# zendesk/min-tfs-client

Hardware: AMD Instinct MI355X
Metric: predict_req_per_s (higher is better)
Workload: dtype fp32; 1 GPU; model=identity-echo[resnet50], global_batch=32, parallelism=dp1, pipeline=4, encoding=turbo, grpc_impl=native, copy_mode=1, streaming=auto, transport=unix, servers_per_rank=1, gpu=True

## Files before the change

min_tfs_client_amd/ops/csrc/grpc_transport.cpp:

```cpp
#include <pybind11/eval.h>
#include <pybind11/functional.h>
#include <pybind11/pybind11.h>
#include <pybind11/stl.h>
#include <torch/extension.h>

#include <c10/hip/HIPCachingAllocator.h>
#include <c10/hip/HIPGuard.h>
#include <c10/hip/HIPStream.h>

#include <algorithm>
#include <atomic>
#include <chrono>
#include <condition_variable>
#include <cstring>
#include <deque>
#include <map>
#include <memory>
#include <mutex>
#include <set>
#include <string>
#include <thread>
#include <unordered_map>
#include <vector>

#include "h2core.h"
#include "hpack.h"
#include "staging.h"
#include "wire.h"

namespace py = pybind11;

namespace {

using h2::Buf;
using h2::Conn;
using h2::ConnError;
using h2::FrameHeader;

struct WireRegion {
  size_t offset;
  size_t nbytes;
  uintptr_t ptr;
  bool device;
};

void write_message_with_regions(Conn& conn, uint32_t stream,
                                const uint8_t* buf, size_t len,
                                const std::vector<WireRegion>& regions,
                                bool end_stream) {
  h2::DataMessageWriter w(conn, stream, len, end_stream);
  size_t pos = 0;
  for (const auto& r : regions) {
    if (r.offset < pos || r.nbytes > len || r.offset > len - r.nbytes)
      throw ConnError("bad streaming region");
    if (r.offset > pos) w.write(buf + pos, r.offset - pos);
    if (!r.device) {
      w.write(reinterpret_cast<const uint8_t*>(r.ptr), r.nbytes);
    } else {
      mi355x_staging::Lease lease;
      lease.ctx->d2h(reinterpret_cast<const void*>(r.ptr), r.nbytes,
                     [&w](const void* chunk, size_t n) {
                       w.write(static_cast<const uint8_t*>(chunk), n);
                     });
    }
    pos = r.offset + r.nbytes;
  }
  if (pos < len) w.write(buf + pos, len - pos);
  w.finish();
}

bool extract_streaming_reply(py::handle result,
                             std::unique_ptr<py::buffer_info>* info,
                             const uint8_t** buf, size_t* len,
                             std::vector<WireRegion>* regions) {
  if (!py::hasattr(result, "_wire_regions")) return false;
  py::object buffer = result.attr("buffer");
  *info = std::make_unique<py::buffer_info>(py::buffer(buffer).request());
  *buf = static_cast<const uint8_t*>((*info)->ptr);
  *len = size_t((*info)->size) * size_t((*info)->itemsize);
  for (auto item : result.attr("_wire_regions")) {
    auto t = py::reinterpret_borrow<py::tuple>(item);
    regions->push_back(WireRegion{
        t[0].cast<size_t>(), t[1].cast<size_t>(),
        uintptr_t(t[2].cast<uint64_t>()), t[3].cast<bool>()});
  }
  return true;
}

struct RpcCallError : std::runtime_error {
  int code;
  RpcCallError(int code_, const std::string& msg)
      : std::runtime_error(msg), code(code_) {}
// ... 121 lines not shown
class ProspectStreams {
 public:
  static ProspectStreams& instance() {
    static ProspectStreams* p = new ProspectStreams();
    return *p;
  }

  static constexpr int kPerDevice = 4;

  hipStream_t get(int device) {
    std::lock_guard<std::mutex> lk(mu_);
    auto it = per_dev_.find(device);
    if (it == per_dev_.end()) {
      std::vector<hipStream_t> v;
      if (hipSetDevice(device) == hipSuccess) {
        for (int i = 0; i < kPerDevice; ++i) {
          hipStream_t s = nullptr;
          if (hipStreamCreateWithFlags(&s, hipStreamNonBlocking) !=
              hipSuccess)
            break;
          v.push_back(s);
        }
      }
      it = per_dev_.emplace(device, std::move(v)).first;
    }
    if (it->second.empty()) return nullptr;
    return it->second[rr_++ % it->second.size()];
  }

 private:
  std::mutex mu_;
  std::unordered_map<int, std::vector<hipStream_t>> per_dev_;
  size_t rr_ = 0;
};

struct DeviceParse {
  bool enabled = false;
  bool failed = false;
  bool done = false;
  int device = 0;
  hipStream_t stream = nullptr;
  int spec_field = 2;
  int map_field = 1;
  std::string spec_name, spec_signature, spec_label;
  int64_t spec_version = -1;
  std::vector<std::string> out_filter;
  std::function<bool(const std::string&)> skip_model;
  size_t pos = 0;
  int state = 0;
  size_t entry_end = 0, tp_end = 0;
  std::string cur_name;
  int cur_dtype = 0;
  std::vector<int64_t> cur_shape;
  bool cur_has_tensor = false;
  at::Tensor cur_tensor;
  bool in_content = false;
  size_t content_off = 0, content_len = 0, content_copied = 0;
  bool copies_issued = false;
  std::vector<std::pair<std::string, at::Tensor>> outs;

  static constexpr size_t kCopyBatch = 1u << 20;

  void fail() {
    failed = true;
    in_content = false;
  }

  void quiesce() {
    if (copies_issued && stream != nullptr) {
      (void)hipStreamSynchronize(stream);
      copies_issued = false;
    }
  }

  DeviceParse() = default;
  DeviceParse(const DeviceParse&) = delete;
  DeviceParse& operator=(const DeviceParse&) = delete;
  DeviceParse(DeviceParse&& o) noexcept { *this = std::move(o); }
  DeviceParse& operator=(DeviceParse&& o) noexcept {
    if (this != &o) {
      quiesce();
      enabled = o.enabled; failed = o.failed; done = o.done;
      device = o.device; stream = o.stream;
      spec_field = o.spec_field; map_field = o.map_field;
      spec_name = std::move(o.spec_name);
      spec_signature = std::move(o.spec_signature);
      spec_label = std::move(o.spec_label);
      spec_version = o.spec_version;
      out_filter = std::move(o.out_filter);
      skip_model = std::move(o.skip_model);
      pos = o.pos; state = o.state;
      entry_end = o.entry_end; tp_end = o.tp_end;
      cur_name = std::move(o.cur_name);
      cur_dtype = o.cur_dtype;
      cur_shape = std::move(o.cur_shape);
      cur_has_tensor = o.cur_has_tensor;
      cur_tensor = std::move(o.cur_tensor);
      in_content = o.in_content;
      content_off = o.content_off;
      content_len = o.content_len;
      content_copied = o.content_copied;
      copies_issued = o.copies_issued;
      outs = std::move(o.outs);
      o.copies_issued = false;
      o.enabled = false;
      o.stream = nullptr;
    }
    return *this;
  }
  ~DeviceParse() { quiesce(); }
};

struct MsgAssembly {
  uint8_t prefix[5];
  size_t prefix_have = 0;
  Buf msg;
  size_t msg_have = 0;
  bool have_len = false;

  void feed_from_socket(int fd, size_t n) {
    while (n > 0) {
      if (prefix_have < 5) {
        size_t take = 5 - prefix_have < n ? 5 - prefix_have : n;
        h2::read_full(fd, prefix + prefix_have, take);
        prefix_have += take;
        n -= take;
        if (prefix_have == 5) {
          if (prefix[0] != 0)
            throw RpcCallError(GRPC_UNIMPLEMENTED,
                               "compressed gRPC messages not supported");
          uint32_t len = h2::be32(prefix + 1);
          if (len > (1u << 30))
            throw RpcCallError(
                GRPC_RESOURCE_EXHAUSTED,
                "received message larger than max (" +
                    std::to_string(len) + " vs 1073741824)");
          size_t cap = 0;
          auto& pool = PinnedPool::instance();
          uint8_t* pinned = pool.get(len, &cap);
          if (pinned != nullptr)
            msg.adopt(pinned, cap, &PinnedPool::deleter, &pool);
          else
            msg.alloc(len);
          msg.len = len;
          have_len = true;
        }
        continue;
      }
      if (!have_len || msg_have + n > msg.len)
        throw ConnError("DATA overruns gRPC message length");
      h2::read_full(fd, msg.p + msg_have, n);
      msg_have += n;
      n = 0;
    }
  }

  bool complete() const { return have_len && msg_have == msg.len; }
};

inline void device_parse_advance(DeviceParse& dp, MsgAssembly& body) {
  if (!dp.enabled || dp.failed || dp.done) return;
  if (!body.have_len) return;
  if (dp.pos == 0 && dp.outs.empty() && !dp.in_content) {
    if (body.msg.deleter == nullptr || body.msg.len < (1u << 20)) {
      dp.enabled = false;
      return;
    }
  }
  const uint8_t* base = body.msg.p;
  const size_t watermark = body.msg_have;
  const size_t total = body.msg.len;

  auto issue_copies = [&]() -> bool {
    size_t span_end = dp.content_off + dp.content_len;
    size_t have_end = watermark < span_end ? watermark : span_end;
    size_t done_abs = dp.content_off + dp.content_copied;
    if (have_end > done_abs) {
      size_t n = have_end - done_abs;
      bool flush = have_end == span_end || body.complete();
      if (n >= DeviceParse::kCopyBatch || flush) {
        if (hipSetDevice(dp.device) != hipSuccess) { dp.fail(); return false; }
        char* dst = static_cast<char*>(dp.cur_tensor.data_ptr())
                    + dp.content_copied;
        if (hipMemcpyAsync(dst, base + done_abs, n, hipMemcpyHostToDevice,
                           dp.stream) != hipSuccess) {
          dp.fail();
          return false;
        }
        dp.copies_issued = true;
        dp.content_copied += n;
      }
    }
    return dp.content_copied == dp.content_len;
  };

  try {
    while (true) {
      if (dp.in_content) {
// ... 62 lines not shown
            tfswire::Cursor v = c.read_len_delim();
            dp.out_filter.emplace_back(
                reinterpret_cast<const char*>(v.p), size_t(v.end - v.p));
            dp.pos = size_t(c.p - base);
          } else {
            dp.fail();
            return;
          }
        } else if (dp.state == 1) {
          int wt = 0;
          int f = c.read_tag(&wt);
          if (f != 1 || wt != tfswire::WT_LEN) { dp.fail(); return; }
          tfswire::Cursor key = c.read_len_delim();
          dp.cur_name.assign(reinterpret_cast<const char*>(key.p),
                             size_t(key.end - key.p));
          f = c.read_tag(&wt);
          if (f != 2 || wt != tfswire::WT_LEN) { dp.fail(); return; }
          uint64_t len = c.read_varint();
          size_t body_off = size_t(c.p - base);
          if (body_off + len > dp.entry_end) { dp.fail(); return; }
          dp.tp_end = body_off + len;
          dp.pos = body_off;
          dp.state = 2;
          dp.cur_dtype = 0;
          dp.cur_shape.clear();
          dp.cur_has_tensor = false;
          dp.cur_tensor = at::Tensor();
        } else {
          if (dp.pos == dp.tp_end) {
            if (!dp.cur_has_tensor) {
              int64_t numel = 1;
              for (int64_t d : dp.cur_shape) numel *= d;
              at::ScalarType st;
              if (numel == 0 && tf_dtype_to_scalar(dp.cur_dtype, &st)) {
                c10::hip::HIPStreamGuard g(c10::hip::getStreamFromExternal(
                    dp.stream, static_cast<c10::DeviceIndex>(dp.device)));
                dp.cur_tensor = at::empty(
                    dp.cur_shape, at::TensorOptions().dtype(st).device(
                                      at::kCUDA, dp.device));
                dp.cur_has_tensor = true;
              } else {
                dp.fail();
                return;
              }
            }
            dp.outs.emplace_back(dp.cur_name, dp.cur_tensor);
            dp.cur_tensor = at::Tensor();
            if (dp.pos != dp.entry_end) { dp.fail(); return; }
            dp.state = 0;
            continue;
          }
          int wt = 0;
          int f = c.read_tag(&wt);
          if (f == 1 && wt == tfswire::WT_VARINT) {
            dp.cur_dtype = int(c.read_varint());
          } else if (f == 2 && wt == tfswire::WT_LEN) {
            tfswire::Cursor sh = c.read_len_delim();
            dp.cur_shape.clear();
            while (!sh.done()) {
              int swt = 0;
              int sf = sh.read_tag(&swt);
              if (sf == 2 && swt == tfswire::WT_LEN) {
                tfswire::Cursor dim = sh.read_len_delim();
                int64_t size = 0;
                while (!dim.done()) {
                  int dwt = 0;
                  int df = dim.read_tag(&dwt);
                  if (df == 1 && dwt == tfswire::WT_VARINT)
                    size = int64_t(dim.read_varint());
                  else
                    dim.skip(dwt);
                }
                dp.cur_shape.push_back(size);
              } else if (sf == 3) {
                dp.fail();
                return;
              } else {
                sh.skip(swt);
              }
            }
          } else if (f == 3 && wt == tfswire::WT_VARINT) {
            (void)c.read_varint();
          } else if (f == 4 && wt == tfswire::WT_LEN) {
            uint64_t len = c.read_varint();
            size_t off = size_t(c.p - base);
            if (off + len > dp.tp_end) { dp.fail(); return; }
            at::ScalarType st;
            if (!tf_dtype_to_scalar(dp.cur_dtype, &st)) { dp.fail(); return; }
            int64_t numel = 1;
            for (int64_t d : dp.cur_shape) numel *= d;
            size_t esize = at::elementSize(st);
            if (uint64_t(numel) * esize != len) { dp.fail(); return; }
            {
              c10::hip::HIPStreamGuard g(c10::hip::getStreamFromExternal(
                  dp.stream, static_cast<c10::DeviceIndex>(dp.device)));
              dp.cur_tensor = at::empty(
                  dp.cur_shape,
                  at::TensorOptions().dtype(st).device(at::kCUDA,
                                                       dp.device));
            }
            dp.content_off = off;
            dp.content_len = size_t(len);
            dp.content_copied = 0;
            dp.in_content = true;
            dp.pos = off;
            continue;
          } else {
            dp.fail();
            return;
          }
          dp.pos = size_t(c.p - base);
        }
      } catch (const std::exception&) {
        (void)step_start;
        if (body.complete()) dp.fail();
        return;
      }
    }
  } catch (...) {
    dp.fail();
  }
}

struct HeaderBlock {
  std::string block;
  bool end_stream = false;
// ... 841 lines not shown
      std::string block = make_request_headers(path, timeout_s);
      try {
        conn_->send_headers(id, block, false);
      } catch (const std::exception& e) {
        pending_.erase(id);
        conn_->close_send_stream(id);
        throw RpcCallError(GRPC_UNAVAILABLE, e.what());
      }
    }
    return id;
  }

  uint32_t start_call(const std::string& path, const uint8_t* data,
                      size_t len, double timeout_s) {
    uint32_t id = begin_stream(path, timeout_s);
    try {
      conn_->send_data_message(id, data, len, true);
    } catch (const std::exception& e) {
      std::lock_guard<std::mutex> lk(mu_);
      pending_.erase(id);
      conn_->close_send_stream(id);
      throw RpcCallError(GRPC_UNAVAILABLE, e.what());
    }
    return id;
  }

  hipStream_t device_stream(int dev) {
    return ProspectStreams::instance().get(dev);
  }

  uint32_t start_call_streaming(const std::string& path, const uint8_t* buf,
                                size_t len,
                                const std::vector<WireRegion>& regions,
                                double timeout_s, int parse_device = -1) {
    uint32_t id = begin_stream(path, timeout_s);
    if (parse_device >= 0) {
      hipStream_t ds = device_stream(parse_device);
      if (ds != nullptr) {
        auto p = find_pending(id);
        if (p) {
          std::lock_guard<std::mutex> lk(p->m);
          p->dparse.enabled = true;
          p->dparse.device = parse_device;
          p->dparse.stream = ds;
        }
      }
    }
    try {
      write_message_with_regions(*conn_, id, buf, len, regions, true);
    } catch (const std::exception& e) {
      std::lock_guard<std::mutex> lk(mu_);
      pending_.erase(id);
      conn_->close_send_stream(id);
      throw RpcCallError(GRPC_UNAVAILABLE, e.what());
    }
    return id;
  }

  struct ParsedResult {
    Buf resp;
    bool parsed_ok = false;
    std::vector<std::pair<std::string, at::Tensor>> outs;
  };

  ParsedResult wait_parsed(uint32_t id, double timeout_s) {
    std::shared_ptr<Pending> p;
    {
      std::lock_guard<std::mutex> lk(mu_);
      auto it = pending_.find(id);
      if (it == pending_.end())
        throw RpcCallError(GRPC_INTERNAL, "unknown call handle");
      p = it->second;
    }
    auto quiesce = [&] {
      std::lock_guard<std::mutex> lk(p->m);
      if (p->dparse.enabled && p->dparse.stream != nullptr)
        (void)hipStreamSynchronize(p->dparse.stream);
    };
    std::unique_lock<std::mutex> lk(p->m);
    bool ok = true;
    if (timeout_s > 0) {
      ok = p->cv.wait_for(lk, std::chrono::duration<double>(timeout_s),
                          [&] { return p->done; });
    } else {
      p->cv.wait(lk, [&] { return p->done; });
    }
    if (!ok) {
      lk.unlock();
      quiesce();
      {
        std::lock_guard<std::mutex> glk(mu_);
        pending_.erase(id);
      }
      try {
        conn_->send_rst_stream(id, 8 );
      } catch (...) {
      }
      conn_->close_send_stream(id);
      cv_.notify_all();
      throw RpcCallError(GRPC_DEADLINE_EXCEEDED, "Deadline Exceeded");
    }
    ParsedResult r;
    r.resp = std::move(p->body.msg);
    int status = p->grpc_status;
    std::string msg = p->message;
    bool parsed = p->dparse.enabled && !p->dparse.failed && p->dparse.done;
    if (parsed) r.outs = std::move(p->dparse.outs);
    bool need_sync = p->dparse.enabled && p->dparse.stream != nullptr;
    hipStream_t ds = p->dparse.stream;
    lk.unlock();
    if (need_sync && hipStreamSynchronize(ds) != hipSuccess) parsed = false;
    if (parsed) record_consumer_stream(r.outs, r.outs.empty() ? 0 :
        r.outs.front().second.get_device());
    {
      std::lock_guard<std::mutex> glk(mu_);
      pending_.erase(id);
    }
    conn_->close_send_stream(id);
    cv_.notify_all();
    if (status != GRPC_OK)
      throw RpcCallError(status < 0 ? GRPC_INTERNAL : status, msg);
    r.parsed_ok = parsed;
    return r;
  }

  Buf wait(uint32_t id, double timeout_s) {
    std::shared_ptr<Pending> p;
    {
      std::lock_guard<std::mutex> lk(mu_);
      auto it = pending_.find(id);
      if (it == pending_.end())
        throw RpcCallError(GRPC_INTERNAL, "unknown call handle");
      p = it->second;
    }
    std::unique_lock<std::mutex> lk(p->m);
    bool ok = true;
    if (timeout_s > 0) {
      ok = p->cv.wait_for(lk, std::chrono::duration<double>(timeout_s),
                          [&] { return p->done; });
    } else {
      p->cv.wait(lk, [&] { return p->done; });
    }
    if (!ok) {
      lk.unlock();
      {
        std::lock_guard<std::mutex> glk(mu_);
        pending_.erase(id);
      }
      try {
        conn_->send_rst_stream(id, 8 );
      } catch (...) {
      }
      conn_->close_send_stream(id);
      cv_.notify_all();
      throw RpcCallError(GRPC_DEADLINE_EXCEEDED, "Deadline Exceeded");
    }
// ... 194 lines not shown
          }
          case h2::F_WINDOW_UPDATE: {
            uint8_t buf4[4];
            if (fh.length != 4) throw ConnError("bad WINDOW_UPDATE");
            h2::read_full(conn_->fd, buf4, 4);
            conn_->apply_window_update(fh.stream,
                                       h2::be32(buf4) & 0x7fffffff);
            break;
          }
          case h2::F_RST_STREAM: {
            uint8_t buf4[4];
            if (fh.length != 4) throw ConnError("bad RST_STREAM");
            h2::read_full(conn_->fd, buf4, 4);
            auto p = find_pending(fh.stream);
            if (p)
              complete(p, GRPC_UNAVAILABLE,
                       "stream reset by server (http2 code " +
                           std::to_string(h2::be32(buf4)) + ")");
            break;
          }
          case h2::F_GOAWAY:
          default:
            h2::discard(conn_->fd, fh.length);
            break;
        }
      }
    } catch (const std::exception& e) {
      conn_->mark_broken(e.what());
      fail_all_pending(GRPC_UNAVAILABLE,
                       std::string("connection lost: ") + e.what());
    }
  }
};

}


PYBIND11_MODULE(_transport, m) {
  m.doc() = "Native gRPC (HTTP/2) transport for the MI355X serving stack";

  py::class_<OwnedBuf>(m, "OwnedBuf", py::buffer_protocol())
      .def_buffer([](OwnedBuf& b) -> py::buffer_info {
        return py::buffer_info(b.buf.p, 1,
                               py::format_descriptor<uint8_t>::format(),
                               1, {py::ssize_t(b.buf.len)}, {py::ssize_t(1)},
                               true );
      })
      .def("__len__", [](const OwnedBuf& b) { return b.buf.len; })
      .def("tobytes", [](const OwnedBuf& b) {
        return py::bytes(reinterpret_cast<const char*>(b.buf.p), b.buf.len);
      });

  static py::object rpc_error_cls = [&m]() {
    py::dict ns;
    py::exec(R"(
class NativeRpcError(Exception):
    """gRPC call failure from the native transport (code_int, details)."""
    def __init__(self, code, details):
        super().__init__(code, details)
        self.code_int = code
        self.details = details
)",
             ns, ns);
    py::object cls = ns["NativeRpcError"];
    m.attr("NativeRpcError") = cls;
    return cls;
// ... 149 lines not shown
                  t[0].cast<size_t>(), t[1].cast<size_t>(),
                  uintptr_t(t[2].cast<uint64_t>()), t[3].cast<bool>()});
            }
            py::gil_scoped_release release;
            return ch.start_call_streaming(path, ptr, len, regions,
                                           timeout, parse_device);
          },
          py::arg("path"), py::arg("data"), py::arg("regions"),
          py::arg("timeout") = 0.0, py::arg("parse_device") = -1,
          "Streaming-region variant of start(); the send completes before "
          "this returns (region memory may be released), the response is "
          "collected with wait().")
      .def(
          "start",
          [](GrpcChannel& ch, const std::string& path, py::buffer data,
             double timeout) {
            py::buffer_info info = data.request();
            const uint8_t* ptr = static_cast<const uint8_t*>(info.ptr);
            size_t len = size_t(info.size) * size_t(info.itemsize);
            py::gil_scoped_release release;
            return ch.start_call(path, ptr, len, timeout);
          },
          py::arg("path"), py::arg("data"), py::arg("timeout") = 0.0)
      .def(
          "wait",
          [](GrpcChannel& ch, uint32_t id, double timeout) {
            py::gil_scoped_release release;
            Buf resp = ch.wait(id, timeout);
            return OwnedBuf(std::move(resp));
          },
          py::arg("id"), py::arg("timeout") = 0.0)
      .def("close", &GrpcChannel::close,
           py::call_guard<py::gil_scoped_release>());
}
```

min_tfs_client_amd/ops/csrc/staging.h:

```cpp
#pragma once

#include <hip/hip_runtime_api.h>

#include <chrono>
#include <condition_variable>
#include <cstdint>
#include <cstdio>
#include <cstdlib>
#include <cstring>
#include <mutex>
#include <stdexcept>
#include <string>
#include <utility>
#include <vector>

namespace mi355x_staging {

#define MI355X_STAGING_CHECK(expr)                                       \
  do {                                                                   \
    hipError_t _e = (expr);                                              \
    if (_e != hipSuccess)                                                \
      throw std::runtime_error(std::string("HIP error in staging: ") +   \
                               hipGetErrorString(_e) + " at " #expr);    \
  } while (0)

inline size_t chunk_size() {
  static const size_t v = [] {
    const char* e = std::getenv("MI355X_STAGING_CHUNK");
    long long n = e ? std::atoll(e) : 0;
    if (n < (1 << 20) || n > (32 << 20)) n = 4 << 20;
    return size_t(n);
  }();
  return v;
}
constexpr int kMaxCtx = 8;

struct Ctx {
  hipStream_t stream = nullptr;
  void* buf[2] = {nullptr, nullptr};
  hipEvent_t evt[2] = {};
  hipEvent_t producer_evt = {};

  void init() {
    MI355X_STAGING_CHECK(
        hipStreamCreateWithFlags(&stream, hipStreamNonBlocking));
    for (int i = 0; i < 2; ++i) {
      MI355X_STAGING_CHECK(hipHostMalloc(&buf[i], chunk_size()));
      MI355X_STAGING_CHECK(
          hipEventCreateWithFlags(&evt[i], hipEventDisableTiming));
    }
    MI355X_STAGING_CHECK(
        hipEventCreateWithFlags(&producer_evt, hipEventDisableTiming));
  }

  void wait_producer(hipStream_t producer) {
    MI355X_STAGING_CHECK(hipEventRecord(producer_evt, producer));
    MI355X_STAGING_CHECK(hipStreamWaitEvent(stream, producer_evt, 0));
  }

  template <typename Consume>
  void d2h(const void* src_dev, size_t nbytes, Consume&& consume) {
    const size_t kChunk = chunk_size();
    size_t nchunks = (nbytes + kChunk - 1) / kChunk;
    const char* trace_path = std::getenv("MI355X_STAGING_TRACE");
    std::vector<double> wait_ms, consume_ms;
    size_t issued = 0;
    for (size_t c = 0; c < (nchunks < 2 ? nchunks : 2); ++c) {
      size_t off = c * kChunk;
      size_t len = nbytes - off < kChunk ? nbytes - off : kChunk;
      MI355X_STAGING_CHECK(hipMemcpyAsync(
          buf[c & 1], static_cast<const char*>(src_dev) + off, len,
          hipMemcpyDeviceToHost, stream));
      MI355X_STAGING_CHECK(hipEventRecord(evt[c & 1], stream));
      ++issued;
    }
    for (size_t c = 0; c < nchunks; ++c) {
      size_t off = c * kChunk;
      size_t len = nbytes - off < kChunk ? nbytes - off : kChunk;
      std::chrono::steady_clock::time_point t0, t1, t2;
      if (trace_path) t0 = std::chrono::steady_clock::now();
      MI355X_STAGING_CHECK(hipEventSynchronize(evt[c & 1]));
      if (trace_path) t1 = std::chrono::steady_clock::now();
      consume(static_cast<const void*>(buf[c & 1]), len);
      if (trace_path) {
        t2 = std::chrono::steady_clock::now();
        wait_ms.push_back(
            std::chrono::duration<double, std::milli>(t1 - t0).count());
        consume_ms.push_back(
            std::chrono::duration<double, std::milli>(t2 - t1).count());
      }
// ... 99 lines not shown
```

min_tfs_client_amd/turbo.py:

```python
from __future__ import annotations

import os
from typing import Dict, Optional, Union

import grpc

try:
    import torch
except ImportError:
    torch = None

from .ops import require_native
from .utils.allocator import tune_malloc
from .utils.metrics import MetricsRegistry
from .utils.tracing import trace_span

_PREDICT_PATH = "/tensorflow.serving.PredictionService/Predict"

_CHANNEL_OPTS = [
    ("grpc.max_send_message_length", 1 << 30),
    ("grpc.max_receive_message_length", 1 << 30),
    ("grpc.http2.max_frame_size", 16 * 1024 * 1024 - 1),
]


def _identity(x: bytes) -> bytes:
    return x


_INT_TO_STATUS = {code.value[0]: code for code in grpc.StatusCode}


class NativeRpcError(grpc.RpcError):

# ... 156 lines not shown
        targets = [target] if isinstance(target, str) else list(target)
        n = max(len(targets), max(1, num_channels))
        self._channels = []
        self._stubs = []
        if backend == "native":
            if credentials is not None:
                raise ValueError("backend='native' is cleartext (h2c); use "
                                 "backend='grpcio' for TLS")
            from . import _transport
            for i in range(n):
                ch = _transport.GrpcChannel(targets[i % len(targets)])
                self._channels.append(ch)
                self._stubs.append(_NativeStub(ch, _PREDICT_PATH))
        elif backend == "grpcio":
            opts = _CHANNEL_OPTS + (options or [])
            for i in range(n):
                copts = opts + [("grpc.use_local_subchannel_pool", 1),
                                ("grpc.channel_id", i)]
                tgt = targets[i % len(targets)]
                if credentials:
                    ch = grpc.secure_channel(tgt, credentials,
                                             options=copts)
                else:
                    ch = grpc.insecure_channel(tgt, options=copts)
                self._channels.append(ch)
                self._stubs.append(ch.unary_unary(
                    _PREDICT_PATH, request_serializer=_identity,
                    response_deserializer=_identity))
        else:
            raise ValueError(f"unknown backend {backend!r}")
        self._channel = self._channels[0]
        self._predict = self._stubs[0]
        self._rr = 0
        self.metrics = MetricsRegistry()
        self.__send_pool = None

    @property
    def _send_pool(self):
        if self.__send_pool is None:
            from concurrent.futures import ThreadPoolExecutor
            self.__send_pool = ThreadPoolExecutor(
                max_workers=16, thread_name_prefix="turbo-send")
        return self.__send_pool

    def _next_stub(self):
        stub = self._stubs[self._rr % len(self._stubs)]
        self._rr += 1
        return stub

    def close(self):
        if self.__send_pool is not None:
            self.__send_pool.shutdown(wait=False)
            self.__send_pool = None
        for ch in self._channels:
            ch.close()

    def __enter__(self):
        return self

    def __exit__(self, *exc):
        self.close()

    def serialize_request(self, model_name: str,
                          inputs: Dict[str, "torch.Tensor"],
                          model_version: Optional[int] = None,
                          signature_name: str = "",
# ... 138 lines not shown
                                signature_name, output_device, copy_mode,
                                streaming=streaming)
        keys = list(inputs.keys())
        if any(inputs[k].dim() == 0 for k in keys):
            return self.predict(model_name, inputs, timeout, model_version,
                                signature_name, output_device, copy_mode,
                                streaming=streaming)
        batch = inputs[keys[0]].shape[0]
        if any(inputs[k].shape[0] != batch for k in keys) \
                or batch < shards:
            return self.predict(model_name, inputs, timeout, model_version,
                                signature_name, output_device, copy_mode,
                                streaming=streaming)
        base, rem = divmod(batch, shards)
        sizes = [base + (1 if i < rem else 0) for i in range(shards)]
        use_streaming = (self.backend == "native" if streaming is None
                         else streaming)
        if use_streaming and self.backend != "native":
            raise ValueError("streaming=True requires backend='native'")

        shard_views = []
        off = 0
        for n in sizes:
            shard_views.append({k: inputs[k].narrow(0, off, n)
                                for k in keys})
            off += n

        dev = str(output_device) if output_device is not None else "cpu"
        parse_dev = -1
        if (use_streaming and dev.startswith("cuda") and torch is not None
                and os.environ.get("MI355X_RX_PARSE", "1") != "0"):
            parse_dev = torch.device(dev).index or 0

        def send_shard(i):
            shard = shard_views[i]
            stub = self._stubs[i % len(self._stubs)]
            if use_streaming:
                blob, regions, keepalive = self._serialize_streaming(
                    model_name, shard, model_version, signature_name)
                if parse_dev >= 0:
                    return stub.future_streaming_parsed(
                        blob, regions, parse_dev, timeout)
                return stub.future_streaming(blob, regions, timeout)
            blob = self.serialize_request(model_name, shard, model_version,
                                          signature_name, copy_mode)
            return stub.future(blob, timeout)

        if self.backend == "native" and shards > 1:
            sends = [self._send_pool.submit(send_shard, i)
                     for i in range(shards)]
            futs = [s.result() for s in sends]
        else:
            futs = [send_shard(i) for i in range(shards)]
        parts = []
        try:
            for fut in futs:
                if isinstance(fut, _NativeParsedFuture):
                    outs, raw = fut.result_parsed()
                    if outs is None:
                        _s, outs, _ = self._native.parse_predict_response(
                            raw, dev, copy_mode)
                    parts.append(outs)
                else:
                    _s, outputs, _ = self._native.parse_predict_response(
                        fut.result(), dev, copy_mode)
                    parts.append(outputs)
        except Exception:
            for fut in futs:
                fut.cancel()
            raise
        merged = {}
        for k in parts[0]:
            vals = [p[k] for p in parts]
            if isinstance(vals[0], torch.Tensor) and vals[0].dim() > 0:
                merged[k] = torch.cat(vals, dim=0)
            else:
                merged[k] = vals[0]
        return merged

    def predict_future(self, model_name, inputs, timeout=60.0,
                       model_version=None, signature_name="",
                       copy_mode: int = 1):
        if self.backend == "native":
            blob, regions, keepalive = self._serialize_streaming(
                model_name, inputs, model_version, signature_name)
            fut = self._next_stub().future_streaming(blob, regions, timeout)
            del keepalive
        else:
            blob = self.serialize_request(model_name, inputs, model_version,
                                          signature_name, copy_mode)
            fut = self._next_stub().future(blob, timeout)

        def decode(resp_bytes, output_device="cpu"):
            _s, outputs, _ = self._native.parse_predict_response(
                resp_bytes, str(output_device), copy_mode)
            return outputs

        return fut, decode
```

Baseline: 776.0 req/s.

## Move sharded predict into native C++ with direct gather into preallocated output

Adds a native predict_sharded path that plans and writes per-shard request skeletons in C++, sends them from a C++ sender thread pool, and has the receive-side device parser write each shard's rows directly into one preallocated full-batch output tensor. This avoids Python-level per-shard serialization, ThreadPoolExecutor dispatch and a final torch.cat. Producer synchronization changes from per-region stream event recording to a single recorded event per device. It adds complexity around failure and cancellation handling and a shared gather target guarded by a mutex.

```diff
diff --git a/min_tfs_client_amd/ops/csrc/grpc_transport.cpp b/min_tfs_client_amd/ops/csrc/grpc_transport.cpp
--- a/min_tfs_client_amd/ops/csrc/grpc_transport.cpp
+++ b/min_tfs_client_amd/ops/csrc/grpc_transport.cpp
@@ -14,6 +14,7 @@
 #include <condition_variable>
 #include <cstring>
 #include <deque>
+#include <functional>
 #include <map>
 #include <memory>
 #include <mutex>
@@ -25,6 +26,7 @@
 
 #include "h2core.h"
 #include "hpack.h"
+#include "shard_plan.h"
 #include "staging.h"
 #include "wire.h"
 
@@ -37,17 +39,14 @@
 using h2::ConnError;
 using h2::FrameHeader;
 
-struct WireRegion {
-  size_t offset;
-  size_t nbytes;
-  uintptr_t ptr;
-  bool device;
-};
+using WireRegion = shardplan::Region;
 
 void write_message_with_regions(Conn& conn, uint32_t stream,
                                 const uint8_t* buf, size_t len,
                                 const std::vector<WireRegion>& regions,
-                                bool end_stream) {
+                                bool end_stream,
+                                const std::vector<hipEvent_t>* producers =
+                                    nullptr) {
   h2::DataMessageWriter w(conn, stream, len, end_stream);
   size_t pos = 0;
   for (const auto& r : regions) {
@@ -58,6 +57,8 @@
       w.write(reinterpret_cast<const uint8_t*>(r.ptr), r.nbytes);
     } else {
       mi355x_staging::Lease lease;
+      if (producers != nullptr)
+        for (hipEvent_t e : *producers) lease.ctx->wait_producer(e);
       lease.ctx->d2h(reinterpret_cast<const void*>(r.ptr), r.nbytes,
                      [&w](const void* chunk, size_t n) {
                        w.write(static_cast<const uint8_t*>(chunk), n);
@@ -245,6 +246,75 @@
   std::mutex mu_;
   std::unordered_map<int, std::vector<hipStream_t>> per_dev_;
   size_t rr_ = 0;
+};
+
+struct GatherTarget {
+  struct Out {
+    std::string name;
+    at::ScalarType st;
+    std::vector<int64_t> rest;
+    at::Tensor full;
+    int taken = 0;
+  };
+
+  std::mutex m;
+  int64_t batch = 0;
+  int device = 0;
+  hipStream_t stream = nullptr;
+  std::atomic<bool> failed{false};
+  std::vector<Out> outs;
+
+  void fail() { failed.store(true, std::memory_order_release); }
+  bool ok() const { return !failed.load(std::memory_order_acquire); }
+
+  at::Tensor take(const std::string& name, at::ScalarType st,
+                  const std::vector<int64_t>& shape, int64_t rows,
+                  int64_t row_off) {
+    std::lock_guard<std::mutex> lk(m);
+    if (!ok()) return at::Tensor();
+    if (shape.empty() || shape[0] != rows || row_off < 0 ||
+        row_off + rows > batch) {
+      fail();
+      return at::Tensor();
+    }
+    Out* o = nullptr;
+    for (auto& e : outs)
+      if (e.name == name) o = &e;
+    if (o == nullptr) {
+      Out e;
+      e.name = name;
+      e.st = st;
+      e.rest.assign(shape.begin() + 1, shape.end());
+      std::vector<int64_t> full_shape = shape;
+      full_shape[0] = batch;
+      try {
+        c10::hip::HIPStreamGuard g(c10::hip::getStreamFromExternal(
+            stream, static_cast<c10::DeviceIndex>(device)));
+        e.full = at::empty(full_shape, at::TensorOptions().dtype(st).device(
+                                           at::kCUDA, device));
+      } catch (...) {
+        fail();
+        return at::Tensor();
+      }
+      outs.push_back(std::move(e));
+      o = &outs.back();
+    } else if (o->st != st || o->rest.size() + 1 != shape.size() ||
+               !std::equal(o->rest.begin(), o->rest.end(),
+                           shape.begin() + 1)) {
+      fail();
+      return at::Tensor();
+    }
+    ++o->taken;
+    return o->full.narrow(0, row_off, rows);
+  }
+
+  bool complete(int shards) {
+    std::lock_guard<std::mutex> lk(m);
+    if (!ok() || outs.empty()) return false;
+    for (auto& e : outs)
+      if (e.taken != shards) return false;
+    return true;
+  }
 };
 
 struct DeviceParse {
@@ -271,12 +341,15 @@
   size_t content_off = 0, content_len = 0, content_copied = 0;
   bool copies_issued = false;
   std::vector<std::pair<std::string, at::Tensor>> outs;
+  std::shared_ptr<GatherTarget> gather;
+  int64_t gather_rows = 0, gather_off = 0;
 
   static constexpr size_t kCopyBatch = 1u << 20;
 
   void fail() {
     failed = true;
     in_content = false;
+    if (gather) gather->fail();
   }
 
   void quiesce() {
@@ -315,6 +388,9 @@
       content_copied = o.content_copied;
       copies_issued = o.copies_issued;
       outs = std::move(o.outs);
+      gather = std::move(o.gather);
+      gather_rows = o.gather_rows;
+      gather_off = o.gather_off;
       o.copies_issued = false;
       o.enabled = false;
       o.stream = nullptr;
@@ -377,6 +453,7 @@
   if (dp.pos == 0 && dp.outs.empty() && !dp.in_content) {
     if (body.msg.deleter == nullptr || body.msg.len < (1u << 20)) {
       dp.enabled = false;
+      if (dp.gather) dp.gather->fail();
       return;
     }
   }
@@ -505,7 +582,8 @@
               int64_t numel = 1;
               for (int64_t d : dp.cur_shape) numel *= d;
               at::ScalarType st;
-              if (numel == 0 && tf_dtype_to_scalar(dp.cur_dtype, &st)) {
+              if (numel == 0 && !dp.gather &&
+                  tf_dtype_to_scalar(dp.cur_dtype, &st)) {
                 c10::hip::HIPStreamGuard g(c10::hip::getStreamFromExternal(
                     dp.stream, static_cast<c10::DeviceIndex>(dp.device)));
                 dp.cur_tensor = at::empty(
@@ -564,7 +642,11 @@
             for (int64_t d : dp.cur_shape) numel *= d;
             size_t esize = at::elementSize(st);
             if (uint64_t(numel) * esize != len) { dp.fail(); return; }
-            {
+            if (dp.gather) {
+              dp.cur_tensor = dp.gather->take(dp.cur_name, st, dp.cur_shape,
+                                              dp.gather_rows, dp.gather_off);
+              if (!dp.cur_tensor.defined()) { dp.fail(); return; }
+            } else {
               c10::hip::HIPStreamGuard g(c10::hip::getStreamFromExternal(
                   dp.stream, static_cast<c10::DeviceIndex>(dp.device)));
               dp.cur_tensor = at::empty(
@@ -1472,10 +1554,15 @@
   uint32_t start_call_streaming(const std::string& path, const uint8_t* buf,
                                 size_t len,
                                 const std::vector<WireRegion>& regions,
-                                double timeout_s, int parse_device = -1) {
+                                double timeout_s, int parse_device = -1,
+                                std::shared_ptr<GatherTarget> gather = nullptr,
+                                int64_t gather_rows = 0,
+                                int64_t gather_off = 0,
+                                const std::vector<hipEvent_t>* producers =
+                                    nullptr) {
     uint32_t id = begin_stream(path, timeout_s);
     if (parse_device >= 0) {
-      hipStream_t ds = device_stream(parse_device);
+      hipStream_t ds = gather ? gather->stream : device_stream(parse_device);
       if (ds != nullptr) {
         auto p = find_pending(id);
         if (p) {
@@ -1483,11 +1570,15 @@
           p->dparse.enabled = true;
           p->dparse.device = parse_device;
           p->dparse.stream = ds;
+          p->dparse.gather = std::move(gather);
+          p->dparse.gather_rows = gather_rows;
+          p->dparse.gather_off = gather_off;
         }
       }
     }
     try {
-      write_message_with_regions(*conn_, id, buf, len, regions, true);
+      write_message_with_regions(*conn_, id, buf, len, regions, true,
+                                 producers);
     } catch (const std::exception& e) {
       std::lock_guard<std::mutex> lk(mu_);
       pending_.erase(id);
@@ -1503,7 +1594,8 @@
     std::vector<std::pair<std::string, at::Tensor>> outs;
   };
 
-  ParsedResult wait_parsed(uint32_t id, double timeout_s) {
+  ParsedResult wait_parsed(uint32_t id, double timeout_s,
+                           bool sync_stream = true) {
     std::shared_ptr<Pending> p;
     {
       std::lock_guard<std::mutex> lk(mu_);
@@ -1527,7 +1619,7 @@
     }
     if (!ok) {
       lk.unlock();
-      quiesce();
+      if (sync_stream) quiesce();
       {
         std::lock_guard<std::mutex> glk(mu_);
         pending_.erase(id);
@@ -1548,10 +1640,16 @@
     if (parsed) r.outs = std::move(p->dparse.outs);
     bool need_sync = p->dparse.enabled && p->dparse.stream != nullptr;
     hipStream_t ds = p->dparse.stream;
+    if (!sync_stream) {
+      need_sync = p->dparse.copies_issued && ds != nullptr &&
+                  status != GRPC_OK;
+      p->dparse.copies_issued = false;
+    }
     lk.unlock();
     if (need_sync && hipStreamSynchronize(ds) != hipSuccess) parsed = false;
-    if (parsed) record_consumer_stream(r.outs, r.outs.empty() ? 0 :
-        r.outs.front().second.get_device());
+    if (parsed && sync_stream)
+      record_consumer_stream(r.outs, r.outs.empty() ? 0 :
+          r.outs.front().second.get_device());
     {
       std::lock_guard<std::mutex> glk(mu_);
       pending_.erase(id);
@@ -1562,6 +1660,19 @@
       throw RpcCallError(status < 0 ? GRPC_INTERNAL : status, msg);
     r.parsed_ok = parsed;
     return r;
+  }
+
+  void cancel_call(uint32_t id) {
+    {
+      std::lock_guard<std::mutex> lk(mu_);
+      pending_.erase(id);
+    }
+    try {
+      conn_->send_rst_stream(id, 8 );
+    } catch (...) {
+    }
+    conn_->close_send_stream(id);
+    cv_.notify_all();
   }
 
   Buf wait(uint32_t id, double timeout_s) {
@@ -1822,6 +1933,286 @@
     }
   }
 };
+
+
+class SenderPool {
+ public:
+  static SenderPool& instance() {
+    static SenderPool* p = new SenderPool();
+    return *p;
+  }
+
+  static constexpr size_t kMaxThreads = 16;
+
+  void submit(std::function<void()> fn) {
+    std::lock_guard<std::mutex> lk(mu_);
+    q_.push_back(std::move(fn));
+    if (q_.size() > idle_ && threads_ < kMaxThreads) {
+      ++threads_;
+      std::thread([this] { loop(); }).detach();
+    }
+    cv_.notify_one();
+  }
+
+ private:
+  void loop() {
+    std::unique_lock<std::mutex> lk(mu_);
+    while (true) {
+      ++idle_;
+      cv_.wait(lk, [this] { return !q_.empty(); });
+      --idle_;
+      std::function<void()> fn = std::move(q_.front());
+      q_.pop_front();
+      lk.unlock();
+      fn();
+      lk.lock();
+    }
+  }
+
+  std::mutex mu_;
+  std::condition_variable cv_;
+  std::deque<std::function<void()>> q_;
+  size_t idle_ = 0, threads_ = 0;
+};
+
+class EventPool {
+ public:
+  static EventPool& instance() {
+    static EventPool* p = new EventPool();
+    return *p;
+  }
+
+  hipEvent_t get(int device) {
+    {
+      std::lock_guard<std::mutex> lk(mu_);
+      auto& fl = free_[device];
+      if (!fl.empty()) {
+        hipEvent_t e = fl.back();
+        fl.pop_back();
+        return e;
+      }
+    }
+    c10::hip::HIPGuard g(static_cast<c10::DeviceIndex>(device));
+    hipEvent_t e = nullptr;
+    if (hipEventCreateWithFlags(&e, hipEventDisableTiming) != hipSuccess)
+      throw RpcCallError(GRPC_INTERNAL, "hipEventCreate failed");
+    return e;
+  }
+
+  void put(int device, hipEvent_t e) {
+    std::lock_guard<std::mutex> lk(mu_);
+    free_[device].push_back(e);
+  }
+
+ private:
+  std::mutex mu_;
+  std::unordered_map<int, std::vector<hipEvent_t>> free_;
+};
+
+struct PooledEvent {
+  int device;
+  hipEvent_t e;
+  explicit PooledEvent(int dev)
+      : device(dev), e(EventPool::instance().get(dev)) {}
+  ~PooledEvent() { EventPool::instance().put(device, e); }
+  PooledEvent(const PooledEvent&) = delete;
+  PooledEvent& operator=(const PooledEvent&) = delete;
+};
+
+inline int scalar_to_tf_dtype(at::ScalarType t) {
+  switch (t) {
+    case at::kFloat: return 1;
+    case at::kDouble: return 2;
+    case at::kInt: return 3;
+    case at::kByte: return 4;
+    case at::kShort: return 5;
+    case at::kChar: return 6;
+    case at::kComplexFloat: return 8;
+    case at::kLong: return 9;
+    case at::kBool: return 10;
+    case at::kBFloat16: return 14;
+    case at::kUInt16: return 17;
+    case at::kComplexDouble: return 18;
+    case at::kHalf: return 19;
+    case at::kUInt32: return 22;
+    case at::kUInt64: return 23;
+    default:
+      throw std::runtime_error("unsupported torch dtype for TensorProto");
+  }
+}
+
+struct ShardedResult {
+  bool gathered = false;
+  std::vector<std::pair<std::string, at::Tensor>> outs;
+  std::vector<Buf> raws;
+  size_t tx_bytes = 0;
+};
+
+ShardedResult predict_sharded_call(
+    const std::vector<GrpcChannel*>& channels, size_t first,
+    const std::string& path, const std::string& model_name, int64_t version,
+    const std::string& signature, const std::vector<std::string>& names,
+    const std::vector<at::Tensor>& tensors, int shards, int parse_device,
+    double timeout_s) {
+  if (channels.empty() || names.size() != tensors.size() || tensors.empty())
+    throw std::invalid_argument("predict_sharded: bad arguments");
+  std::vector<shardplan::Input> inputs(tensors.size());
+  for (size_t i = 0; i < tensors.size(); ++i) {
+    const at::Tensor& t = tensors[i];
+    if (t.dim() == 0 || !t.is_contiguous())
+      throw std::invalid_argument("predict_sharded: input not shardable");
+    inputs[i].name = names[i];
+    inputs[i].dtype = scalar_to_tf_dtype(t.scalar_type());
+    inputs[i].shape.assign(t.sizes().begin(), t.sizes().end());
+    inputs[i].elem_size = size_t(t.element_size());
+    inputs[i].base = static_cast<const uint8_t*>(t.const_data_ptr());
+    inputs[i].device = t.is_cuda();
+  }
+  const int64_t batch = inputs[0].shape[0];
+  for (auto& in : inputs)
+    if (in.shape[0] != batch)
+      throw std::invalid_argument("predict_sharded: dim 0 mismatch");
+  const std::vector<int64_t> sizes = shardplan::shard_sizes(batch, shards);
+  const std::vector<int64_t> offs = shardplan::shard_offsets(sizes);
+
+  std::vector<std::unique_ptr<PooledEvent>> producer_evts;
+  std::vector<hipEvent_t> producers;
+  for (auto& t : tensors) {
+    if (!t.is_cuda()) continue;
+    int dev = int(t.get_device());
+    bool have = false;
+    for (auto& pe : producer_evts) have = have || pe->device == dev;
+    if (have) continue;
+    producer_evts.push_back(std::make_unique<PooledEvent>(dev));
+    c10::hip::HIPGuard g(static_cast<c10::DeviceIndex>(dev));
+    if (hipEventRecord(producer_evts.back()->e,
+                       c10::hip::getCurrentHIPStream(
+                           static_cast<c10::DeviceIndex>(dev))
+                           .stream()) != hipSuccess)
+      throw RpcCallError(GRPC_INTERNAL, "hipEventRecord failed");
+    producers.push_back(producer_evts.back()->e);
+  }
+
+  std::shared_ptr<GatherTarget> gather;
+  hipStream_t ds = nullptr;
+  if (parse_device >= 0) {
+    ds = ProspectStreams::instance().get(parse_device);
+    if (ds != nullptr) {
+      gather = std::make_shared<GatherTarget>();
+      gather->batch = batch;
+      gather->device = parse_device;
+      gather->stream = ds;
+    }
+  }
+  auto drain = [&] {
+    if (gather) gather->fail();
+    if (ds != nullptr) {
+      c10::hip::HIPGuard g(static_cast<c10::DeviceIndex>(parse_device));
+      (void)hipStreamSynchronize(ds);
+    }
+  };
+
+  struct Shard {
+    Buf skel;
+    std::vector<WireRegion> regions;
+    GrpcChannel* ch = nullptr;
+    uint32_t id = 0;
+    bool started = false;
+    std::exception_ptr err;
+  };
+  std::vector<Shard> sh;
+  sh.resize(size_t(shards));
+  ShardedResult res;
+  for (int i = 0; i < shards; ++i) {
+    auto sp = shardplan::plan_shard(model_name, version, signature, inputs,
+                                    offs[size_t(i)], sizes[size_t(i)]);
+    Shard& s = sh[size_t(i)];
+    s.skel.alloc(size_t(sp.plan.total_size));
+    s.skel.len = size_t(sp.plan.total_size);
+    s.regions = shardplan::write_shard(s.skel.p, sp, model_name, version,
+                                       signature, inputs);
+    s.ch = channels[(first + size_t(i)) % channels.size()];
+    res.tx_bytes += size_t(sp.plan.total_size);
+  }
+
+  const bool have_producers = !producers.empty();
+  auto send_one = [&](int i) {
+    Shard& s = sh[size_t(i)];
+    try {
+      s.id = s.ch->start_call_streaming(
+          path, s.skel.p, s.skel.len, s.regions, timeout_s, parse_device,
+          gather, sizes[size_t(i)], offs[size_t(i)],
+          have_producers ? &producers : nullptr);
+      s.started = true;
+    } catch (...) {
+      s.err = std::current_exception();
+    }
+  };
+  {
+    std::mutex lm;
+    std::condition_variable lcv;
+    int outstanding = shards - 1;
+    for (int i = 1; i < shards; ++i) {
+      SenderPool::instance().submit([&, i] {
+        send_one(i);
+        std::lock_guard<std::mutex> lk(lm);
+        if (--outstanding == 0) lcv.notify_one();
+      });
+    }
+    send_one(0);
+    std::unique_lock<std::mutex> lk(lm);
+    lcv.wait(lk, [&] { return outstanding == 0; });
+  }
+  for (int i = 0; i < shards; ++i) {
+    if (!sh[size_t(i)].err) continue;
+    for (auto& s : sh)
+      if (s.started) s.ch->cancel_call(s.id);
+    drain();
+    std::rethrow_exception(sh[size_t(i)].err);
+  }
+
+  bool all_parsed = gather != nullptr;
+  res.raws.resize(size_t(shards));
+  std::vector<size_t> nouts(size_t(shards), 0);
+  for (int i = 0; i < shards; ++i) {
+    Shard& s = sh[size_t(i)];
+    try {
+      if (parse_device >= 0) {
+        GrpcChannel::ParsedResult r =
+            s.ch->wait_parsed(s.id, timeout_s, !gather);
+        res.raws[size_t(i)] = std::move(r.resp);
+        all_parsed = all_parsed && r.parsed_ok;
+        nouts[size_t(i)] = r.outs.size();
+      } else {
+        res.raws[size_t(i)] = s.ch->wait(s.id, timeout_s);
+      }
+    } catch (...) {
+      for (int j = i + 1; j < shards; ++j)
+        sh[size_t(j)].ch->cancel_call(sh[size_t(j)].id);
+      drain();
+      throw;
+    }
+  }
+  if (!gather) return res;
+
+  {
+    c10::hip::HIPGuard g(static_cast<c10::DeviceIndex>(parse_device));
+    PooledEvent done(parse_device);
+    if (hipEventRecord(done.e, ds) != hipSuccess ||
+        hipEventSynchronize(done.e) != hipSuccess) {
+      drain();
+      all_parsed = false;
+    }
+  }
+  if (all_parsed && gather->complete(shards)) {
+    for (size_t n : nouts)
+      if (n != gather->outs.size()) return res;
+    for (auto& o : gather->outs) res.outs.emplace_back(o.name, o.full);
+    record_consumer_stream(res.outs, parse_device);
+    res.gathered = true;
+  }
+  return res;
+}
 
 }
 
@@ -2037,4 +2428,90 @@
           py::arg("id"), py::arg("timeout") = 0.0)
       .def("close", &GrpcChannel::close,
            py::call_guard<py::gil_scoped_release>());
+
+  m.def(
+      "predict_sharded",
+      [](py::list channel_list, size_t first_channel,
+         const std::string& path, const std::string& model_name,
+         int64_t version, const std::string& signature,
+         const std::vector<std::string>& names,
+         const std::vector<at::Tensor>& tensors, int shards,
+         int parse_device, double timeout) {
+        std::vector<GrpcChannel*> channels;
+        channels.reserve(py::len(channel_list));
+        for (auto item : channel_list)
+          channels.push_back(item.cast<GrpcChannel*>());
+        std::vector<at::Tensor> contig;
+        contig.reserve(tensors.size());
+        for (auto& t : tensors) contig.push_back(t.contiguous());
+        ShardedResult r;
+        {
+          py::gil_scoped_release release;
+          r = predict_sharded_call(channels, first_channel, path,
+                                   model_name, version, signature, names,
+                                   contig, shards, parse_device, timeout);
+        }
+        py::object outs = py::none();
+        if (r.gathered) {
+          py::dict d;
+          for (auto& kv : r.outs) d[py::str(kv.first)] = kv.second;
+          outs = std::move(d);
+        }
+        py::list raws;
+        for (auto& b : r.raws) raws.append(OwnedBuf(std::move(b)));
+        return py::make_tuple(outs, raws, r.tx_bytes);
+      },
+      py::arg("channels"), py::arg("first_channel"), py::arg("path"),
+      py::arg("model_name"), py::arg("version"), py::arg("signature"),
+      py::arg("names"), py::arg("tensors"), py::arg("shards"),
+      py::arg("parse_device") = -1, py::arg("timeout") = 0.0,
+      "One logical Predict split along dim 0 into `shards` requests, run "
+      "as a single GIL-free call: shard i rides channels[(first_channel + "
+      "i) % n]. Returns ({name: [batch, ...] device tensor} | None, [raw "
+      "response per shard], request bytes sent); the dict is None when "
+      "the responses could not be gathered in place — parse and "
+      "concatenate the raw buffers instead.");
+
+  m.def(
+      "shard_wire",
+      [](const std::string& model_name, int64_t version,
+         const std::string& signature,
+         const std::vector<std::string>& names,
+         const std::vector<at::Tensor>& tensors, int shards) {
+        std::vector<shardplan::Input> inputs(tensors.size());
+        std::vector<at::Tensor> contig;
+        for (size_t i = 0; i < tensors.size(); ++i) {
+          contig.push_back(tensors[i].contiguous());
+          const at::Tensor& t = contig.back();
+          inputs[i].name = names.at(i);
+          inputs[i].dtype = scalar_to_tf_dtype(t.scalar_type());
+          inputs[i].shape.assign(t.sizes().begin(), t.sizes().end());
+          inputs[i].elem_size = size_t(t.element_size());
+          inputs[i].base = static_cast<const uint8_t*>(t.const_data_ptr());
+          inputs[i].device = t.is_cuda();
+        }
+        if (inputs.empty() || inputs[0].shape.empty())
+          throw std::invalid_argument("shard_wire: need batched inputs");
+        auto sizes = shardplan::shard_sizes(inputs[0].shape[0], shards);
+        auto offs = shardplan::shard_offsets(sizes);
+        py::list out;
+        for (size_t i = 0; i < sizes.size(); ++i) {
+          auto sp = shardplan::plan_shard(model_name, version, signature,
+                                          inputs, offs[i], sizes[i]);
+          std::string buf(size_t(sp.plan.total_size), '\0');
+          auto regions = shardplan::write_shard(
+              reinterpret_cast<uint8_t*>(&buf[0]), sp, model_name, version,
+              signature, inputs);
+          py::list rl;
+          for (auto& r : regions)
+            rl.append(py::make_tuple(uint64_t(r.offset), uint64_t(r.nbytes),
+                                     uint64_t(r.ptr), r.device));
+          out.append(py::make_tuple(py::bytes(buf), rl));
+        }
+        return out;
+      },
+      py::arg("model_name"), py::arg("version"), py::arg("signature"),
+      py::arg("names"), py::arg("tensors"), py::arg("shards"),
+      "Per-shard (skeleton bytes, regions) exactly as predict_sharded "
+      "sends them (shard_plan.h); for tests and diagnostics.");
 }
diff --git a/min_tfs_client_amd/ops/csrc/shard_plan.h b/min_tfs_client_amd/ops/csrc/shard_plan.h
--- /dev/null
+++ b/min_tfs_client_amd/ops/csrc/shard_plan.h
@@ -0,0 +1,123 @@
+#pragma once
+
+#include <algorithm>
+#include <cstdint>
+#include <cstring>
+#include <stdexcept>
+#include <string>
+#include <vector>
+
+#include "wire.h"
+
+namespace shardplan {
+
+constexpr size_t kStreamMinSpan = 64 * 1024;
+
+struct Region {
+  size_t offset;
+  size_t nbytes;
+  uintptr_t ptr;
+  bool device;
+};
+
+struct Input {
+  std::string name;
+  int dtype = 0;
+  std::vector<int64_t> shape;
+  size_t elem_size = 0;
+  const uint8_t* base = nullptr;
+  bool device = false;
+
+  size_t row_bytes() const {
+    size_t n = elem_size;
+    for (size_t d = 1; d < shape.size(); ++d) n *= size_t(shape[d]);
+    return n;
+  }
+};
+
+inline std::vector<int64_t> shard_sizes(int64_t batch, int shards) {
+  if (shards < 1 || batch < shards)
+    throw std::invalid_argument("shard_plan: need 1 <= shards <= batch");
+  int64_t base = batch / shards, rem = batch % shards;
+  std::vector<int64_t> sizes(size_t(shards), base);
+  for (int64_t i = 0; i < rem; ++i) sizes[size_t(i)] += 1;
+  return sizes;
+}
+
+inline std::vector<int64_t> shard_offsets(const std::vector<int64_t>& sizes) {
+  std::vector<int64_t> offs(sizes.size());
+  int64_t off = 0;
+  for (size_t i = 0; i < sizes.size(); ++i) {
+    offs[i] = off;
+    off += sizes[i];
+  }
+  return offs;
+}
+
+struct ShardPlan {
+  int64_t rows = 0;
+  int64_t row_off = 0;
+  std::vector<std::string> names;
+  std::vector<tfswire::TensorMeta> metas;
+  tfswire::SkeletonPlan plan;
+};
+
+inline ShardPlan plan_shard(const std::string& model_name, int64_t version,
+                            const std::string& signature,
+                            const std::vector<Input>& inputs,
+                            int64_t row_off, int64_t rows) {
+  ShardPlan sp;
+  sp.rows = rows;
+  sp.row_off = row_off;
+  sp.names.reserve(inputs.size());
+  sp.metas.resize(inputs.size());
+  for (size_t i = 0; i < inputs.size(); ++i) {
+    const Input& in = inputs[i];
+    if (in.shape.empty() || row_off < 0 || rows < 0 ||
+        row_off + rows > in.shape[0])
+      throw std::invalid_argument("shard_plan: rows outside input '" +
+                                  in.name + "'");
+    sp.names.push_back(in.name);
+    sp.metas[i].dtype = in.dtype;
+    sp.metas[i].shape = in.shape;
+    sp.metas[i].shape[0] = rows;
+    sp.metas[i].content_bytes = uint64_t(rows) * in.row_bytes();
+    if (sp.metas[i].content_bytes >= (uint64_t(1) << 31))
+      throw std::invalid_argument(
+          "tensor '" + in.name + "' exceeds the 2GB tensor_content limit "
+          "of the protobuf wire format");
+  }
+  sp.plan = tfswire::plan_predict_message(true, model_name, version,
+                                          signature, sp.names, sp.metas);
+  return sp;
+}
+
+inline std::vector<Region> write_shard(uint8_t* buf, ShardPlan& sp,
+                                       const std::string& model_name,
+                                       int64_t version,
+                                       const std::string& signature,
+                                       const std::vector<Input>& inputs) {
+  tfswire::write_predict_message(buf, sp.plan, true, model_name, version,
+                                 signature, sp.names, sp.metas);
+  std::vector<size_t> order(inputs.size());
+  for (size_t i = 0; i < order.size(); ++i) order[i] = i;
+  std::sort(order.begin(), order.end(), [&](size_t a, size_t b) {
+    return sp.plan.spans[a].offset < sp.plan.spans[b].offset;
+  });
+  std::vector<Region> regions;
+  for (size_t idx : order) {
+    const auto& span = sp.plan.spans[idx];
+    if (span.nbytes == 0) continue;
+    const Input& in = inputs[idx];
+    const uint8_t* src = in.base + size_t(sp.row_off) * in.row_bytes();
+    if (in.device || span.nbytes >= kStreamMinSpan) {
+      regions.push_back(Region{size_t(span.offset), size_t(span.nbytes),
+                               reinterpret_cast<uintptr_t>(src), in.device});
+    } else {
+      std::memcpy(buf + span.offset, src, span.nbytes);
+    }
+  }
+  return regions;
+}
+
+}
diff --git a/min_tfs_client_amd/ops/csrc/staging.h b/min_tfs_client_amd/ops/csrc/staging.h
--- a/min_tfs_client_amd/ops/csrc/staging.h
+++ b/min_tfs_client_amd/ops/csrc/staging.h
@@ -56,6 +56,10 @@
   void wait_producer(hipStream_t producer) {
     MI355X_STAGING_CHECK(hipEventRecord(producer_evt, producer));
     MI355X_STAGING_CHECK(hipStreamWaitEvent(stream, producer_evt, 0));
+  }
+
+  void wait_producer(hipEvent_t recorded) {
+    MI355X_STAGING_CHECK(hipStreamWaitEvent(stream, recorded, 0));
   }
 
   template <typename Consume>
diff --git a/min_tfs_client_amd/turbo.py b/min_tfs_client_amd/turbo.py
--- a/min_tfs_client_amd/turbo.py
+++ b/min_tfs_client_amd/turbo.py
@@ -1,5 +1,6 @@
 from __future__ import annotations
 
+import itertools
 import os
 from typing import Dict, Optional, Union
 
@@ -222,6 +223,7 @@
         self._channel = self._channels[0]
         self._predict = self._stubs[0]
         self._rr = 0
+        self._shard_rr = itertools.count()
         self.metrics = MetricsRegistry()
         self.__send_pool = None
 
@@ -426,6 +428,12 @@
                 and os.environ.get("MI355X_RX_PARSE", "1") != "0"):
             parse_dev = torch.device(dev).index or 0
 
+        if (use_streaming
+                and os.environ.get("MI355X_NATIVE_SHARDED", "1") != "0"):
+            return self._predict_sharded_native(
+                model_name, inputs, keys, shards, timeout, model_version,
+                signature_name, dev, parse_dev, copy_mode)
+
         def send_shard(i):
             shard = shard_views[i]
             stub = self._stubs[i % len(self._stubs)]
@@ -472,6 +480,34 @@
                 merged[k] = vals[0]
         return merged
 
+    @_translate_native_error
+    def _predict_sharded_native(self, model_name, inputs, keys, shards,
+                                timeout, model_version, signature_name,
+                                dev, parse_dev, copy_mode):
+        from . import _transport
+        first = 0
+        if os.environ.get("MI355X_SHARD_ROTATE", "1") != "0":
+            first = next(self._shard_rr) * shards
+        outs, raws, tx_bytes = _transport.predict_sharded(
+            self._channels, first % len(self._channels), _PREDICT_PATH,
+            model_name, -1 if model_version is None else model_version,
+            signature_name, keys, [inputs[k] for k in keys], shards,
+            parse_dev, timeout or 0.0)
+        self.metrics.observe_bytes("tx", tx_bytes)
+        self.metrics.observe_bytes("rx", sum(len(r) for r in raws))
+        if outs is not None:
+            return outs
+        parts = [self._native.parse_predict_response(raw, dev, copy_mode)[1]
+                 for raw in raws]
+        merged = {}
+        for k in parts[0]:
+            vals = [p[k] for p in parts]
+            if isinstance(vals[0], torch.Tensor) and vals[0].dim() > 0:
+                merged[k] = torch.cat(vals, dim=0)
+            else:
+                merged[k] = vals[0]
+        return merged
+
     def predict_future(self, model_name, inputs, timeout=60.0,
                        model_version=None, signature_name="",
                        copy_mode: int = 1):
```

Measured after the change: 853.8 req/s (median of 6 runs). +10.0%, better.
